# AppleHolic/pytorch_sound

Hardware: AMD Instinct MI355X
Metric: audio-sec/s STFT+mel+fwd/bwd (higher is better)
Workload: dtype bf16; 1 GPU; configs[1]: Conv1d separator (4 x ResBlock1, C=256, on 513-bin magnitude), 22.05 kHz, STFT 1024/256, 80 mel, batch 32 x 2 s per GPU, Adam, bf16 autocast; global_batch=32, parallelism=dp1, model_params=5520386

## Files before the change

include/psnd.h:

```cpp
#ifndef PSND_H
#define PSND_H

#include <stdint.h>
#include <stddef.h>

#ifdef __cplusplus
extern "C" {
#endif

#define PSND_OK 0
#define PSND_E_ARG (-1)
#define PSND_E_SHAPE (-2)
#define PSND_E_HIP (-3)
#define PSND_E_UNSUPPORTED (-4)

#define PSND_FRAMING_CENTER 0
#define PSND_FRAMING_HIFIGAN 1
#define PSND_FRAMING_NONE 2

int psnd_version(void);
const char *psnd_last_error(void);
#ifdef PSND_LAB
void psnd_env_refresh(void);
#endif
// ... 89 lines not shown
typedef struct psnd_chain_pair {
    const void *W1;
    const float *bias1;
    float act1_slope;
    void *mid_out;
    const void *W2;
    const float *bias2;
    int off1, dstep1, off2, dstep2;
    float act2_slope;
    void *out_raw, *out_act;
    const void *M1, *M2;
    float m1_slope, m2_slope;
} psnd_chain_pair;
int psnd_conv1d_cl_chain_rows(int C, int k, int n_pairs, const int *taps);
int psnd_conv1d_cl_chain_plan(int C, int k, int n_pairs, const int *taps, int64_t R, int *mr_out);
int psnd_conv1d_cl_chain(const void *A, const void *res, const psnd_chain_pair *pairs, int n_pairs, int64_t N, int Lp, int L, int HP,
                         int C, int k, void *stream);
void psnd_conv_chain_stats(long long *out2);
int psnd_to_cl_nfk(const float *x_nfk, int64_t N, int K, int64_t F, int Lp, int HP, int Cp, int preop, void *out, void *stream);
int64_t psnd_mask_head_l1_blocks_nfk(int64_t N, int64_t F, int K);
int psnd_mask_head_l1_fwd_nfk(const void *y, const float *mag_nfk, const float *ref_nfk, int64_t N, int K, int64_t F, int Lp, int HP, int Cp,
                              float *est_nfk, double *part, void *stream);
int psnd_mask_head_l1_bwd_nfk(const float *gest_nfk, const float *mag_nfk, const void *y, const float *est_nfk, const float *ref_nfk,
                              const float *g, float coef, int64_t N, int K, int64_t F, int Lp, int HP, int Cp, void *gy, void *stream);
int psnd_mel_fwd_nfk(const float *mag_nfk, int64_t N, int64_t F, int M, int K, const void *mel_plan, int log_kind, float log_offset,
                     float pre_clamp_min, float clamp_lo, float clamp_hi, float *out, float *mel_lin, void *stream);
int psnd_mel_bwd_nfk(const float *gout, const float *mel_lin, int64_t N, int64_t F, int M, int K, const void *mel_plan, int log_kind,
                     float log_offset, float pre_clamp_min, float clamp_lo, float clamp_hi, float *gmag_nfk, void *stream);
int psnd_mel_l1_fwd_nfk(const float *mag_nfk, int64_t N, int64_t F, int M, int K, const void *mel_plan, int log_kind, float log_offset,
                        float pre_clamp_min, float clamp_lo, float clamp_hi, const float *ref, float *mel_lin, double *part, void *stream);
int psnd_mel_l1_bwd_nfk(const float *ref, const float *mel_lin, const float *g, float coef, int64_t N, int64_t F, int M, int K,
                        const void *mel_plan, int log_kind, float log_offset, float pre_clamp_min, float clamp_lo, float clamp_hi,
                        float *gmag_nfk, void *stream);
int64_t psnd_mask_head_l1_blocks(int64_t N, int64_t T, int Cp);
int psnd_mask_head_l1_fwd(const void *y, const float *mag, const float *ref, int64_t N, int C, int64_t T, int Lp, int HP, int Cp,
                          float *est, double *part, void *stream);
int psnd_mask_head_l1_bwd(const float *gest, const float *mag, const void *y, const float *est, const float *ref, const float *g,
                          float coef, int64_t N, int C, int64_t T, int Lp, int HP, int Cp, void *gy, void *stream);
int64_t psnd_mel_l1_blocks(int64_t N, int64_t F, int M);
int psnd_mel_l1_fwd(const float *mag, int64_t N, int64_t F, int M, int K, const void *mel_plan, int log_kind, float log_offset,
                    float pre_clamp_min, float clamp_lo, float clamp_hi, const float *ref, float *mel_lin, double *part, void *stream);
int psnd_mel_l1_bwd(const float *ref, const float *mel_lin, const float *g, float coef, int64_t N, int64_t F, int M, int K,
                    const void *mel_plan, int log_kind, float log_offset, float pre_clamp_min, float clamp_lo, float clamp_hi,
                    float *gmag, void *stream);
int psnd_nan_flag(const float *x, int64_t n, float *flag, void *stream);
int psnd_l1_loss_combine(const double *const *parts, const int64_t *nb, const double *scale, int terms, float *out, float *nan_flag, void *stream);
int psnd_conv_stats(int64_t *out4, int reset);
int psnd_conv_pair_stats(int64_t *out4, int reset);
int psnd_conv1d_cl_wgrad(const void *G1, const void *G2, const void *GM, float g2_slope, const void *xa, int64_t N,
                         int Lp, int Ca, int Cb, int k, int off0, int dstep, float *gw_part, float *gbias_part,
                         void *g_out, void *stream);
int psnd_conv1d_prep(const float *v, const float *g, const float *bias, int Cout, int Cin, int k, int Cb, int Ca,
                     void *wf, void *wb, float *bias_padded, void *stream);
int psnd_convtr1d_prep(const float *v, const float *g, const float *bias, int Cin, int Cout, int K, int stride, int Cr, int Cip,
                       void *wf, void *wb, float *bias_rep, void *stream);
int psnd_convtr1d_prep_multi(const void *descs_dev, int n, int total_blocks, void *stream);
int psnd_convtr1d_cl_fwd(const void *xa, const void *wf, const float *bias_rep, int64_t N, int Lp, int L, int HP, int Cip, int Cr,
                         int stride, int padding, int LpO, int HPO, float act_slope, void *out_raw, void *out_act, void *stream);
int psnd_convtr1d_cl_wgrad_splits(int64_t N, int Lp, int Cip, int Cr, int stride);
int psnd_convtr1d_cl_bwd(const void *g_raw, const void *g_act, const void *act, float act_slope, const void *wb, const void *xa,
                         int64_t N, int Lp, int L, int HP, int Cip, int Cr, int stride, int padding, int LpO, int HPO, void *gx,
                         void *g_eff, float *gw_part, void *stream);
int psnd_convtr1d_wnorm_bwd(const float *gw_part, int splits, const float *v, const float *g, int Cin, int Cout, int K, int stride,
                            int Cr, int Cip, float *gv, float *gg, void *stream);
int psnd_cl_mean_act_fwd(const void *a, const void *b, const void *c, const void *d, int count, float slope, void *out, int64_t n,
                         void *stream);
// ... 175 lines not shown
```

pytorch_sound_amd/_lib.py:

```python
import ctypes
import os
import numpy as np

_HERE = os.path.dirname(os.path.abspath(__file__))
LIB_PATH = os.environ.get('PSND_LIB', os.path.join(_HERE, 'libpsnd_hip.so'))

PSND_OK = 0
FRAMING_CENTER = 0
FRAMING_HIFIGAN = 1
FRAMING_NONE = 2
LOG_NONE, LOG_E, LOG_10 = 0, 1, 2
MASK_NONE, MASK_LINEAR, MASK_SIGMOID = 0, 1, 2

_c = ctypes
_P = _c.c_void_p
_I64 = _c.c_int64
_INT = _c.c_int
_F = _c.c_float
_D = _c.c_double
_U32 = _c.c_uint32
_U64 = _c.c_uint64

SIGNATURES = {
    'psnd_version': (_INT, []),
# ... 30 lines not shown
    'psnd_conv1d_cl': (_INT, [_P, _P, _P, _F, _P, _P, _P, _P, _I64, _INT, _INT, _INT, _INT, _INT, _INT, _INT, _INT, _F, _F, _P, _P, _P, _P]),
    'psnd_conv1d_cl_pair_supported': (_INT, [_INT, _INT, _INT, _INT, _INT, _INT]),
    'psnd_conv1d_cl_pair': (_INT, [_P, _P, _P, _P, _F, _F, _P, _P, _P, _P, _F, _P, _I64, _INT, _INT, _INT, _INT, _INT, _INT, _INT, _INT, _INT, _F, _P, _P, _P]),
    'psnd_conv1d_cl_wgrad': (_INT, [_P, _P, _P, _F, _P, _I64, _INT, _INT, _INT, _INT, _INT, _INT, _P, _P, _P, _P]),
    'psnd_conv1d_prep': (_INT, [_P, _P, _P, _INT, _INT, _INT, _INT, _INT, _P, _P, _P, _P]),
    'psnd_conv1d_wnorm_bwd': (_INT, [_P, _P, _INT, _P, _P, _INT, _INT, _INT, _INT, _INT, _P, _P, _P, _P]),
    'psnd_conv1d_cl_bwd': (_INT, [_P, _P, _P, _F, _P, _P, _I64, _INT, _INT, _INT, _INT, _INT, _INT, _INT, _INT, _P, _P, _P, _F, _P, _P, _P, _P]),
    'psnd_conv1d_cl_wgrad_multi_splits': (_INT, [_I64, _INT, _INT, _INT, _INT, _INT]),
    'psnd_conv1d_cl_wgrad_multi': (_INT, [_P, _INT, _I64, _INT, _P]),
    'psnd_nan_flag': (_INT, [_P, _I64, _P, _P]),
    'psnd_conv1d_cl_chain_rows': (_INT, [_INT, _INT, _INT, _P]),
    'psnd_conv1d_cl_chain_plan': (_INT, [_INT, _INT, _INT, _P, _I64, _P]),
    'psnd_conv1d_cl_chain': (_INT, [_P, _P, _P, _INT, _I64, _INT, _INT, _INT, _INT, _INT, _P]),
    'psnd_conv_chain_stats': (None, [_P]),
    'psnd_conv1d_cl_pair_bwd_supported': (_INT, [_INT, _INT, _INT, _INT, _INT, _INT]),
    'psnd_conv1d_cl_pair_bwd_splits': (_INT, [_I64, _INT, _INT, _INT]),
    'psnd_conv1d_cl_pair_bwd': (_INT, [_P, _P, _P, _F, _P, _P, _P, _F, _P, _I64, _INT, _INT, _INT, _INT, _INT, _INT, _INT, _INT, _INT, _P, _P, _P, _P,
                                       _P, _P, _INT, _INT, _P, _P, _P]),
    'psnd_conv1d_wnorm_bwd_multi': (_INT, [_P, _INT, _P]),
    'psnd_conv1d_prep_multi': (_INT, [_P, _INT, _INT, _INT, _INT, _P]),
    'psnd_conv1d_cl_wgrad_splits': (_INT, [_I64, _INT, _INT, _INT, _INT]),
    'psnd_mask_head_l1_blocks': (_I64, [_I64, _I64, _INT]),
    'psnd_masked_l1_blocks': (_I64, [_I64]),
    'psnd_masked_l1_fwd': (_INT, [_P, _P, _P, _I64, _INT, _I64, _P, _P, _P, _P]),
    'psnd_masked_l1_bwd': (_INT, [_P, _P, _P, _I64, _INT, _I64, _P, _P, _P, _P, _P]),
    'psnd_to_cl_nfk': (_INT, [_P, _I64, _INT, _I64, _INT, _INT, _INT, _INT, _P, _P]),
    'psnd_mask_head_l1_blocks_nfk': (_I64, [_I64, _I64, _INT]),
    'psnd_mask_head_l1_fwd_nfk': (_INT, [_P, _P, _P, _I64, _INT, _I64, _INT, _INT, _INT, _P, _P, _P]),
    'psnd_mask_head_l1_bwd_nfk': (_INT, [_P, _P, _P, _P, _P, _P, _F, _I64, _INT, _I64, _INT, _INT, _INT, _P, _P]),
    'psnd_mel_fwd_nfk': (_INT, [_P, _I64, _I64, _INT, _INT, _P, _INT, _F, _F, _F, _F, _P, _P, _P]),
    'psnd_mel_bwd_nfk': (_INT, [_P, _P, _I64, _I64, _INT, _INT, _P, _INT, _F, _F, _F, _F, _P, _P]),
    'psnd_mel_l1_fwd_nfk': (_INT, [_P, _I64, _I64, _INT, _INT, _P, _INT, _F, _F, _F, _F, _P, _P, _P, _P]),
    'psnd_mel_l1_bwd_nfk': (_INT, [_P, _P, _P, _F, _I64, _I64, _INT, _INT, _P, _INT, _F, _F, _F, _F, _P, _P]),
    'psnd_mask_head_l1_fwd': (_INT, [_P, _P, _P, _I64, _INT, _I64, _INT, _INT, _INT, _P, _P, _P]),
    'psnd_mask_head_l1_bwd': (_INT, [_P, _P, _P, _P, _P, _P, _F, _I64, _INT, _I64, _INT, _INT, _INT, _P, _P]),
    'psnd_mel_l1_blocks': (_I64, [_I64, _I64, _INT]),
    'psnd_mel_l1_fwd': (_INT, [_P, _I64, _I64, _INT, _INT, _P, _INT, _F, _F, _F, _F, _P, _P, _P, _P]),
    'psnd_mel_l1_bwd': (_INT, [_P, _P, _P, _F, _I64, _I64, _INT, _INT, _P, _INT, _F, _F, _F, _F, _P, _P]),
    'psnd_l1_loss_combine': (_INT, [_P, _P, _P, _INT, _P, _P, _P]),
    'psnd_conv_stats': (_INT, [_P, _INT]),
    'psnd_conv_pair_stats': (_INT, [_P, _INT]),
    'psnd_convtr1d_prep_multi': (_INT, [_P, _INT, _INT, _P]),
    'psnd_convtr1d_prep': (_INT, [_P, _P, _P, _INT, _INT, _INT, _INT, _INT, _INT, _P, _P, _P, _P]),
    'psnd_convtr1d_cl_fwd': (_INT, [_P, _P, _P, _I64, _INT, _INT, _INT, _INT, _INT, _INT, _INT, _INT, _INT, _F, _P, _P, _P]),
    'psnd_convtr1d_cl_wgrad_splits': (_INT, [_I64, _INT, _INT, _INT, _INT]),
    'psnd_convtr1d_cl_bwd': (_INT, [_P, _P, _P, _F, _P, _P, _I64, _INT, _INT, _INT, _INT, _INT, _INT, _INT, _INT, _INT, _P, _P, _P, _P]),
    'psnd_convtr1d_wnorm_bwd': (_INT, [_P, _INT, _P, _P, _INT, _INT, _INT, _INT, _INT, _INT, _P, _P, _P]),
    'psnd_cl_mean_act_fwd': (_INT, [_P, _P, _P, _P, _INT, _F, _P, _I64, _P]),
    'psnd_cl_mean_act_bwd': (_INT, [_P, _P, _INT, _F, _P, _I64, _P]),
    'psnd_cl_sum2': (_INT, [_P, _INT, _P, _P, _INT, _P, _I64, _P]),
    'psnd_grad_pack_bf16': (_INT, [_P, _P, _I64, _F, _P]),
    'psnd_grad_unpack_bf16': (_INT, [_P, _P, _I64, _F, _P]),
    'psnd_cl_colsum_splits': (_INT, [_I64, _INT]),
    'psnd_cl_colsum': (_INT, [_P, _I64, _INT, _INT, _INT, _INT, _P, _P, _P]),
    'psnd_posenc': (_INT, [_P, _P, _F, _I64, _INT, _I64, _I64, _P, _P]),
    'psnd_groupnorm1_fwd': (_INT, [_P, _P, _P, _P, _I64, _INT, _I64, _F, _INT, _P, _P, _P, _P]),
    'psnd_groupnorm1_bwd': (_INT, [_P, _P, _P, _P, _P, _P, _I64, _INT, _I64, _INT, _P, _P, _P, _P, _P]),
    'psnd_groupnorm1_drop_fwd': (_INT, [_P, _P, _P, _P, _I64, _INT, _I64, _F, _INT, _P, _P, _P, _P, _U32, _F, _P]),
    'psnd_groupnorm1_drop_bwd': (_INT, [_P, _P, _P, _P, _P, _P, _I64, _INT, _I64, _INT, _P, _P, _P, _P, _P, _P, _U32, _F, _P]),
    'psnd_rng_seed': (_INT, [_P, _U64, _U64, _P]),
    'psnd_rng_next': (_INT, [_P, _P, _P]),
    'psnd_linear1x1_fwd': (_INT, [_P, _P, _P, _I64, _INT, _INT, _I64, _INT, _INT, _P, _P]),
    'psnd_linear1x1_wgrad_slabs': (_I64, [_I64, _INT, _INT, _I64]),
    'psnd_linear1x1_bwd': (_INT, [_P, _P, _P, _P, _I64, _INT, _INT, _I64, _INT, _P, _P, _P, _P, _P]),
    'psnd_linear1x1_bwd_acc': (_INT, [_P, _P, _P, _P, _I64, _INT, _INT, _I64, _INT, _P, _P, _P, _P, _P, _P]),
    'psnd_linear1x1_bwd_ex': (_INT, [_P, _P, _P, _P, _I64, _INT, _INT, _I64, _INT, _INT, _I64, _P, _P, _P, _P, _P, _P, _P]),
# ... 199 lines not shown
```

pytorch_sound_amd/cl.py:

```python
import ctypes
from collections import namedtuple
from pytorch_sound_amd import _switches as _sw
import weakref

import torch

from . import _lib
from ._lib import lib, check, ptr, stream_ptr

ALIGN_C = 32


def round_up(x, m):
    return (x + m - 1) // m * m


class CLShape:

    def __init__(self, N, L, HP):
        self.N, self.L, self.HP = int(N), int(L), int(HP)
        self.Lp = round_up(self.L + 2 * self.HP, 8)

    @property
    def R(self):
# ... 168 lines not shown
    def backward(ctx, g, _gest):
        y, mag, mag_ref, mel_ref, mel_plan, est, lin = ctx.saved_tensors
        shape, M, log_kind, log_offset, pre, lo, hi, c1, c2 = ctx.cfg
        N, C, T = mag.shape
        if g is None:
            return (None,) * 14
        g = g.contiguous().float()
        gest = torch.empty_like(mag)
        gy = torch.empty_like(y)
        st = stream_ptr(y.device)
        with torch.cuda.device(y.device):
            check(lib().psnd_mel_l1_bwd(ptr(mel_ref), ptr(lin), ptr(g), c2, N, T, M, C, ptr(mel_plan), log_kind, log_offset, pre, lo, hi,
                                        ptr(gest), st), 'psnd_mel_l1_bwd')
            check(lib().psnd_mask_head_l1_bwd(ptr(gest), ptr(mag), ptr(y), ptr(est), ptr(mag_ref), ptr(g), c1, N, C, T, shape.Lp, shape.HP,
                                              y.shape[2], ptr(gy), st), 'psnd_mask_head_l1_bwd')
        return (gy,) + (None,) * 13


def to_cl_nfk(x_nfk, shape, preop=0):
    _need(x_nfk, torch.float32)
    if x_nfk.requires_grad and torch.is_grad_enabled():
        raise _lib.PsndError('to_cl_nfk carries no gradient (feature tensors are inputs); use ToCL on an (N, K, F) tensor')
    N, F, K = x_nfk.shape
    if F != shape.L or N != shape.N:
        raise _lib.PsndError('to_cl_nfk: tensor %s does not match the CL geometry (N=%d, L=%d)' % (tuple(x_nfk.shape), shape.N, shape.L))
    Cp = round_up(K, ALIGN_C)
    out = torch.empty((N, shape.Lp, Cp), dtype=torch.bfloat16, device=x_nfk.device)
    with torch.cuda.device(x_nfk.device):
        check(lib().psnd_to_cl_nfk(ptr(x_nfk), N, K, F, shape.Lp, shape.HP, Cp, int(preop), ptr(out), stream_ptr(x_nfk.device)),
              'psnd_to_cl_nfk')
    return out


class MaskHeadSpectralL1NFK(torch.autograd.Function):

    @staticmethod
    def forward(ctx, y, mag, mag_ref, mel_ref, mel_plan, shape, M, log_kind, log_offset, pre_clamp_min, clamp_lo, clamp_hi, w1, w2):
        from .kernels import _clamp_args
        ctx.set_materialize_grads(False)
        _need(y, torch.bfloat16)
        for t in (mag, mag_ref, mel_ref):
            _need(t, torch.float32)
        N, F, K = mag.shape
        if mag_ref.shape != mag.shape or tuple(mel_ref.shape) != (N, M, F):
            raise _lib.PsndError('mask_head_spectral_l1 (nfk): mag_ref %s / mel_ref %s do not match mag %s and %d mel bands'
                                 % (tuple(mag_ref.shape), tuple(mel_ref.shape), tuple(mag.shape), M))
        dev = y.device
        lo, hi, pre = _clamp_args(clamp_lo, clamp_hi, pre_clamp_min)
        est = torch.empty_like(mag)
        lin = torch.empty((N, M, F), dtype=torch.float32, device=dev)
        nb1 = int(lib().psnd_mask_head_l1_blocks_nfk(N, F, K))
        nb2 = int(lib().psnd_mel_l1_blocks(N, F, M))
        part = torch.empty(nb1 + nb2, dtype=torch.float64, device=dev)
        out = torch.empty((), dtype=torch.float32, device=dev)
        st = stream_ptr(dev)
        with torch.cuda.device(dev):
            check(lib().psnd_mask_head_l1_fwd_nfk(ptr(y), ptr(mag), ptr(mag_ref), N, K, F, shape.Lp, shape.HP, y.shape[2], ptr(est),
                                                  ptr(part), st), 'psnd_mask_head_l1_fwd_nfk')
            p2 = ctypes.c_void_p(part.data_ptr() + 8 * nb1)
            check(lib().psnd_mel_l1_fwd_nfk(ptr(est), N, F, M, K, ptr(mel_plan), log_kind, float(log_offset), pre, lo, hi, ptr(mel_ref),
                                            ptr(lin), p2, st), 'psnd_mel_l1_fwd_nfk')
            parts = (ctypes.c_void_p * 2)(part.data_ptr(), part.data_ptr() + 8 * nb1)
            nbs = (ctypes.c_int64 * 2)(nb1, nb2)
            sc = (ctypes.c_double * 2)(float(w1) / mag.numel(), float(w2) / mel_ref.numel())
            nan_flag = _nan_flag_tensor(dev)
            check(lib().psnd_l1_loss_combine(parts, nbs, sc, 2, ptr(out), ptr(nan_flag), st), 'psnd_l1_loss_combine')
        LAST_LOSS_NAN_FLAG[0] = nan_flag
        ctx.cfg = (shape, M, log_kind, float(log_offset), pre, lo, hi, float(w1) / mag.numel(), float(w2) / mel_ref.numel())
        ctx.save_for_backward(y, mag, mag_ref, mel_ref, mel_plan, est, lin)
        ctx.mark_non_differentiable(est)
        return out, est

    @staticmethod
    def backward(ctx, g, _gest):
        y, mag, mag_ref, mel_ref, mel_plan, est, lin = ctx.saved_tensors
        shape, M, log_kind, log_offset, pre, lo, hi, c1, c2 = ctx.cfg
        N, F, K = mag.shape
        if g is None:
            return (None,) * 14
        g = g.contiguous().float()
        gest = torch.empty_like(mag)
        gy = torch.empty_like(y)
        st = stream_ptr(y.device)
        with torch.cuda.device(y.device):
            check(lib().psnd_mel_l1_bwd_nfk(ptr(mel_ref), ptr(lin), ptr(g), c2, N, F, M, K, ptr(mel_plan), log_kind, log_offset, pre, lo, hi,
                                            ptr(gest), st), 'psnd_mel_l1_bwd_nfk')
            check(lib().psnd_mask_head_l1_bwd_nfk(ptr(gest), ptr(mag), ptr(y), ptr(est), ptr(mag_ref), ptr(g), c1, N, K, F, shape.Lp,
                                                  shape.HP, y.shape[2], ptr(gy), st), 'psnd_mask_head_l1_bwd_nfk')
        return (gy,) + (None,) * 13


def _launch_conv(A, A2, AM, a2_slope, W, bias, res, mask_src, shape, Ca, Cb, k, off0, dstep, act_slope, mask_slope,
                 want_raw, want_act, a_eff_out=None):
    dev = W.device
    raw = torch.empty((shape.N, shape.Lp, Cb), dtype=torch.bfloat16, device=dev) if want_raw else None
    act = torch.empty((shape.N, shape.Lp, Cb), dtype=torch.bfloat16, device=dev) if want_act else None
    with torch.cuda.device(dev):
        check(lib().psnd_conv1d_cl(ptr(A), ptr(A2), ptr(AM), float(a2_slope), ptr(W), ptr(bias), ptr(res), ptr(mask_src),
                                   shape.N, shape.Lp, shape.L, shape.HP, Ca, Cb, k, off0, dstep, float(act_slope),
                                   float(mask_slope), ptr(raw), ptr(act), ptr(a_eff_out), stream_ptr(dev)), 'psnd_conv1d_cl')
    return raw, act


_JOIN_PENDING = {}


def _join_side_at_end_of_backward(dev, side):
    target = torch.cuda.current_stream(dev)
    pending = _JOIN_PENDING.setdefault(dev.index, [])
    if not any(t == target and sd == side for t, sd in pending):
        pending.append((target, side))

    def join():
# ... 968 lines not shown
```

pytorch_sound_amd/csrc/psnd_core.hip:

```cpp
#include "psnd_common.h"

static thread_local char g_err[512] = "";

void psnd_set_error(const char *fmt, ...) {
    va_list ap;
    va_start(ap, fmt);
    vsnprintf(g_err, sizeof(g_err), fmt, ap);
    va_end(ap);
}

extern "C" int psnd_version(void) { return 144; }

extern "C" const char *psnd_last_error(void) { return g_err; }

#ifdef PSND_LAB
std::atomic<int> g_psnd_env_gen{0};
extern "C" void psnd_env_refresh(void) { g_psnd_env_gen.fetch_add(1, std::memory_order_acq_rel); }
#endif

static inline int64_t pad_of(int n_fft, int hop, int framing) {
    if (framing == PSND_FRAMING_NONE) return 0;
    return framing == PSND_FRAMING_CENTER ? n_fft / 2 : (n_fft - hop) / 2;
}

extern "C" int64_t psnd_frame_count(int64_t T, int n_fft, int hop, int framing) {
    if (T <= 0 || n_fft <= 0 || hop <= 0) return 0;
    const int64_t L = T + 2 * pad_of(n_fft, hop, framing);
    if (L < n_fft) return 0;
    return (L - n_fft) / hop + 1;
}

extern "C" int64_t psnd_frame_sample_index(int64_t f, int m, int64_t T, int n_fft, int hop, int framing) {
    int64_t i = f * hop - pad_of(n_fft, hop, framing) + m;
    if (i < 0) i = -i;
    if (i >= T) i = 2 * (T - 1) - i;
    return i;
}

extern "C" void *psnd_event_create(void) {
    hipEvent_t ev = nullptr;
    if (hipEventCreateWithFlags(&ev, hipEventDisableTiming) != hipSuccess) {
        psnd_set_error("event_create: %s", hipGetErrorString(hipGetLastError()));
        return nullptr;
    }
// ... 96 lines not shown
```

pytorch_sound_amd/csrc/psnd_mel.hip:

```cpp
#include "psnd_common.h"
#include <math.h>
#include <string.h>
#include <vector>

namespace {

inline int hdr_ints(int MT, int KT) { return (8 + 2 * MT + 2 * KT + 63) & ~63; }

struct MelParams {
    const float *in0;
    const float *in1;
    const int *plan;
    float *out;
    float *lin;
    long long F;
    int N, R, Cc;
    int RT, CS;
    int band_off;
    int w_off;
    int nft;
    int log_kind;
    float log_offset, pre_clamp_min, clamp_lo, clamp_hi;
    const float *l1_ref;
    double *l1_part;
    const float *l1_g;
    float l1_coef;
    int wn_off, CS16;
    int seg_off;
};

__device__ __forceinline__ float log_grad(float mel, int kind, float off, float pre, float lo, float hi) {
    float pass = 1.f;
    float v = mel;
    if (pre >= 0.f) {
        if (v < pre) pass = 0.f;
        v = fmaxf(v, pre);
    }
    v += off;
    float y = v, d = 1.f;
    if (kind == PSND_LOG_E) {
        y = logf(v);
        d = 1.f / v;
    } else if (kind == PSND_LOG_10) {
        y = log10f(v);
        d = 0.43429448190325182765f / v;
    }
    if (y < lo || y > hi) pass = 0.f;
    return pass * d;
}

__device__ __forceinline__ float l1_log_grad(float mel, float ref, int kind, float off, float pre, float lo, float hi) {
    float pass = 1.f, v = mel;
    if (pre >= 0.f) {
        if (v < pre) pass = 0.f;
        v = fmaxf(v, pre);
    }
    v += off;
    float y = v, d = 1.f;
    if (kind == PSND_LOG_E) {
        y = logf(v);
        d = 1.f / v;
    } else if (kind == PSND_LOG_10) {
        y = log10f(v);
        d = 0.43429448190325182765f / v;
    }
    if (y < lo || y > hi) pass = 0.f;
    y = fminf(fmaxf(y, lo), hi);
    const float sg = y > ref ? 1.f : (y < ref ? -1.f : 0.f);
    return sg * pass * d;
}

__device__ __forceinline__ f32x4 load_b_raw(__amdgpu_buffer_rsrc_t r, int c, int Cc, long long f, long long F) {
    const unsigned off = (c < Cc && f < F) ? (unsigned)(((size_t)c * F + f) * sizeof(float)) : 0xffffffffu;
    return __builtin_bit_cast(f32x4, __builtin_amdgcn_raw_buffer_load_b128(r, (int)off, 0, 0));
}

template <bool BWD, bool NFK = false>
__global__ __launch_bounds__(256) void mel_kernel(MelParams p) {
    const int lane = threadIdx.x & 63;
    const long long wid = (long long)blockIdx.x * 4 + (threadIdx.x >> 6);
    const long long per_clip = (long long)p.nft * p.RT;
    if (wid >= per_clip * p.N) return;
    const int clip = (int)(wid / per_clip);
    const int rem = (int)(wid - (long long)clip * per_clip);
    const int ft = rem / p.RT, rt = rem - ft * p.RT;
    const long long F = p.F;
    const long long f = (long long)ft * 64 + 4 * (lane & 15);
    const int kk = lane >> 4;

    const int lo = p.plan[p.band_off + 2 * rt], hi = p.plan[p.band_off + 2 * rt + 1];
    const float *W = reinterpret_cast<const float *>(p.plan) + p.w_off + (size_t)rt * p.CS * 64 + lane;
    const int in_bytes = (int)((size_t)p.Cc * F * sizeof(float));
    const __amdgpu_buffer_rsrc_t r0 = make_uniform_rsrc(p.in0 + (size_t)clip * p.Cc * F, in_bytes);
    const __amdgpu_buffer_rsrc_t r1 = make_uniform_rsrc(BWD ? p.in1 + (size_t)clip * p.Cc * F : p.in0, BWD ? in_bytes : 0);
    const bool l1b = BWD && p.l1_g != nullptr;
    const float l1c = l1b ? p.l1_coef * p.l1_g[0] : 0.f;

    f32x4 acc0 = {0.f, 0.f, 0.f, 0.f}, acc1 = acc0, acc2 = acc0, acc3 = acc0;
    auto batch = [&](auto muc, int s0) __attribute__((always_inline)) {
        constexpr int MU = decltype(muc)::value;
        float a[MU];
        f32x4 b[MU], m[BWD ? MU : 1];
#pragma unroll
        for (int u = 0; u < MU; ++u) {
            const int c = s0 + u < hi ? 4 * (s0 + u) + kk : p.Cc;
            a[u] = W[(size_t)min(s0 + u, hi - 1) * 64];
            b[u] = load_b_raw(r0, c, p.Cc, f, F);
            if constexpr (BWD) m[u] = load_b_raw(r1, c, p.Cc, f, F);
        }
        if constexpr (BWD) {
// ... 7 lines not shown
                } else {
                    b[u].x *= log_grad(m[u].x, p.log_kind, p.log_offset, p.pre_clamp_min, p.clamp_lo, p.clamp_hi);
                    b[u].y *= log_grad(m[u].y, p.log_kind, p.log_offset, p.pre_clamp_min, p.clamp_lo, p.clamp_hi);
                    b[u].z *= log_grad(m[u].z, p.log_kind, p.log_offset, p.pre_clamp_min, p.clamp_lo, p.clamp_hi);
                    b[u].w *= log_grad(m[u].w, p.log_kind, p.log_offset, p.pre_clamp_min, p.clamp_lo, p.clamp_hi);
                }
                if (!(s0 + u < hi && 4 * (s0 + u) + kk < p.Cc)) b[u] = f32x4{0.f, 0.f, 0.f, 0.f};
            }
        }
#pragma unroll
        for (int u = 0; u < MU; ++u) {
            acc0 = __builtin_amdgcn_mfma_f32_16x16x4f32(a[u], b[u].x, acc0, 0, 0, 0);
            acc1 = __builtin_amdgcn_mfma_f32_16x16x4f32(a[u], b[u].y, acc1, 0, 0, 0);
            acc2 = __builtin_amdgcn_mfma_f32_16x16x4f32(a[u], b[u].z, acc2, 0, 0, 0);
            acc3 = __builtin_amdgcn_mfma_f32_16x16x4f32(a[u], b[u].w, acc3, 0, 0, 0);
        }
    };
#ifndef PSND_MEL_MU
#define PSND_MEL_MU 8
#endif
    constexpr int MU = BWD ? 4 : PSND_MEL_MU;
    int s0 = lo;
    for (; s0 + MU <= hi; s0 += MU) batch(std::integral_constant<int, MU>{}, s0);
    if constexpr (BWD) {
        const int rest = hi - s0;
        if (rest == 1) batch(std::integral_constant<int, 1>{}, s0);
        else if (rest == 2) batch(std::integral_constant<int, 2>{}, s0);
        else if (rest == 3) batch(std::integral_constant<int, 3>{}, s0);
    } else {
        if (s0 < hi) batch(std::integral_constant<int, MU>{}, s0);
    }
    const size_t obase = (size_t)clip * p.R * F;
    float l1acc = 0.f;
    if constexpr (BWD && NFK) {
        const int bin0 = 16 * rt + 4 * kk;
        const f32x4 accs[4] = {acc0, acc1, acc2, acc3};
#pragma unroll
        for (int j = 0; j < 4; ++j) {
            if (f + j >= F || bin0 >= p.R) continue;
            float *dst = p.out + obase + (size_t)(f + j) * p.R + bin0;
            if (bin0 + 3 < p.R) {
                *reinterpret_cast<f32x4_u *>(dst) = accs[j];
            } else {
                for (int r = 0; r < 4; ++r)
                    if (bin0 + r < p.R) dst[r] = accs[j][r];
            }
        }
        return;
    }
#pragma unroll
    for (int r = 0; r < 4; ++r) {
        const int row = 16 * rt + 4 * kk + r;
        if (row >= p.R) continue;
        f32x4 v = {acc0[r], acc1[r], acc2[r], acc3[r]};
        f32x4 y = v;
        if constexpr (!BWD) {
            y.x = fminf(fmaxf(log_apply(v.x, p.log_kind, p.log_offset, p.pre_clamp_min), p.clamp_lo), p.clamp_hi);
            y.y = fminf(fmaxf(log_apply(v.y, p.log_kind, p.log_offset, p.pre_clamp_min), p.clamp_lo), p.clamp_hi);
            y.z = fminf(fmaxf(log_apply(v.z, p.log_kind, p.log_offset, p.pre_clamp_min), p.clamp_lo), p.clamp_hi);
            y.w = fminf(fmaxf(log_apply(v.w, p.log_kind, p.log_offset, p.pre_clamp_min), p.clamp_lo), p.clamp_hi);
        }
        const size_t o = obase + (size_t)row * F + f;
        if constexpr (!BWD) {
            if (p.l1_ref) {
                if (f + 3 < F) {
                    const f32x4 rf = *reinterpret_cast<const f32x4_u *>(p.l1_ref + o);
                    l1acc += fabsf(y.x - rf.x) + fabsf(y.y - rf.y) + fabsf(y.z - rf.z) + fabsf(y.w - rf.w);
// ... 296 lines not shown
            if (any) {
                if (s < lo) lo = s;
                hi = s + 1;
            }
        }
        if (hi <= lo) lo = hi = 0;
        hdr[8 + 2 * h.MT + 2 * t] = lo, hdr[8 + 2 * h.MT + 2 * t + 1] = hi;
    }
    for (int t = 0; t < h.MT; ++t)
        for (int S = 0; S < h.KS16; ++S)
            for (int lane = 0; lane < 64; ++lane)
                for (int j = 0; j < 4; ++j)
                    fl[h.wn_off + (((size_t)t * h.KS16 + S) * 64 + lane) * 4 + j] = w(16 * t + (lane & 15), 16 * S + 4 * (lane >> 4) + j);
    {
        int *sg = hdr + h.seg_off;
        auto lo = [&](int t) { return hdr[8 + 2 * t]; };
        auto hi = [&](int t) { return hdr[8 + 2 * t + 1]; };
        bool banded = true;
        for (int t = 0; t + 1 < h.MT; ++t) banded &= lo(t) <= lo(t + 1) && hi(t) <= hi(t + 1) && hi(t) > lo(t) && hi(t + 1) > lo(t + 1);
        for (int t = 0; t + 2 < h.MT; ++t) banded &= hi(t) <= lo(t + 2);
        for (int t = 0; t < h.MT; ++t) {
            int s1b = lo(t), s1e = hi(t), s2b = 0, s2e = 0;
            if (banded) {
                if (t > 0 && hi(t - 1) > s1b) s1b = hi(t - 1);
                if (t + 1 < h.MT && lo(t + 1) < s1e) s2b = lo(t + 1), s2e = s1e, s1e = s2b;
                if (s1e < s1b) s1e = s1b;
            }
            sg[4 * t] = s1b, sg[4 * t + 1] = s1e, sg[4 * t + 2] = s2b, sg[4 * t + 3] = s2e;
        }
    }
    return PSND_OK;
}

static int mel_launch(bool bwd, const float *in0, const float *in1, int64_t N, int64_t F, int M, int K,
                      const void *plan, int log_kind, float log_offset, float pre, float lo, float hi,
                      float *out, float *lin, void *stream, const float *l1_ref = nullptr, double *l1_part = nullptr,
                      const float *l1_g = nullptr, float l1_coef = 0.f, bool nfk = false) {
    if (!in0 || !plan || (!out && !l1_ref) || (bwd && !in1)) PSND_FAIL(PSND_E_ARG, "mel: null pointer");
    if (M <= 0 || K <= 0 || N < 0 || F < 0) PSND_FAIL(PSND_E_SHAPE, "mel: M=%d K=%d N=%lld F=%lld", M, K, (long long)N, (long long)F);
    if (log_kind < PSND_LOG_NONE || log_kind > PSND_LOG_10) PSND_FAIL(PSND_E_ARG, "mel: log_kind=%d", log_kind);
    if (N == 0 || F == 0) return PSND_OK;
    if ((size_t)(M > K ? M : K) * (size_t)F * sizeof(float) >= ((size_t)1 << 31))
        PSND_FAIL(PSND_E_SHAPE, "mel: a clip of %lld frames exceeds the 2 GB buffer range of one clip's operand", (long long)F);
    const MelHostPlan h = mel_layout(M, K);
    MelParams p;
    p.in0 = in0, p.in1 = in1, p.plan = static_cast<const int *>(plan), p.out = out, p.lin = lin;
    p.F = F, p.N = (int)N;
    p.log_kind = log_kind, p.log_offset = log_offset, p.pre_clamp_min = pre, p.clamp_lo = lo, p.clamp_hi = hi;
    p.nft = (int)((F + 63) / 64);
    p.l1_ref = l1_ref, p.l1_part = l1_part, p.l1_g = l1_g, p.l1_coef = l1_coef;
    p.wn_off = h.wn_off, p.CS16 = h.KS16, p.seg_off = h.seg_off;
    if (!bwd) {
        p.R = M, p.Cc = K, p.RT = h.MT, p.CS = h.KS, p.band_off = 8, p.w_off = h.fw_off;
    } else {
        p.R = K, p.Cc = M, p.RT = h.KT, p.CS = h.MS, p.band_off = 8 + 2 * h.MT, p.w_off = h.bw_off;
    }
    const bool once = !bwd && !nfk && h.MT <= kOnceTiles;
    const long long waves = (long long)N * p.nft * p.RT;
    const long long blocks = (waves + 3) / 4;
    if (blocks >= (1ll << 31) || waves >= (1ll << 31)) PSND_FAIL(PSND_E_SHAPE, "mel: grid too large");
    hipStream_t s = static_cast<hipStream_t>(stream);
    if (nfk) {
        if (!bwd) hipLaunchKernelGGL(mel_fwd_nfk_kernel, dim3((unsigned)waves), dim3(256), 0, s, p);
        else hipLaunchKernelGGL((mel_kernel<true, true>), dim3((unsigned)blocks), dim3(256), 0, s, p);
    } else if (!bwd && once) {
        const long long ob = ((long long)N * p.nft + 3) / 4;
        if (h.MT <= 5) hipLaunchKernelGGL(mel_fwd_once_kernel<5>, dim3((unsigned)ob), dim3(256), 0, s, p);
        else hipLaunchKernelGGL(mel_fwd_once_kernel<8>, dim3((unsigned)ob), dim3(256), 0, s, p);
    } else if (!bwd) hipLaunchKernelGGL(mel_kernel<false>, dim3((unsigned)blocks), dim3(256), 0, s, p);
    else hipLaunchKernelGGL(mel_kernel<true>, dim3((unsigned)blocks), dim3(256), 0, s, p);
    PSND_CHECK_LAUNCH(bwd ? "mel_bwd" : "mel_fwd");
    return PSND_OK;
}

extern "C" int psnd_mel_fwd(const float *mag, int64_t N, int64_t F, int M, int K, const void *mel_plan,
                            int log_kind, float log_offset, float pre_clamp_min, float clamp_lo, float clamp_hi,
                            float *out, float *mel_lin, void *stream) {
    return mel_launch(false, mag, nullptr, N, F, M, K, mel_plan, log_kind, log_offset, pre_clamp_min, clamp_lo,
                      clamp_hi, out, mel_lin, stream);
}

extern "C" int psnd_mel_bwd(const float *gout, const float *mel_lin, int64_t N, int64_t F, int M, int K,
                            const void *mel_plan, int log_kind, float log_offset, float pre_clamp_min,
                            float clamp_lo, float clamp_hi, float *gmag, void *stream) {
    return mel_launch(true, gout, mel_lin, N, F, M, K, mel_plan, log_kind, log_offset, pre_clamp_min, clamp_lo,
                      clamp_hi, gmag, nullptr, stream);
}

extern "C" int64_t psnd_mel_l1_blocks(int64_t N, int64_t F, int M) {
    if (N <= 0 || F <= 0 || M <= 0) return 0;
    return N * ((F + 63) / 64) * ((M + 15) / 16);
}
extern "C" int psnd_mel_l1_fwd(const float *mag, int64_t N, int64_t F, int M, int K, const void *mel_plan, int log_kind, float log_offset,
                               float pre_clamp_min, float clamp_lo, float clamp_hi, const float *ref, float *mel_lin, double *part,
                               void *stream) {
    if (!ref || !mel_lin || !part) PSND_FAIL(PSND_E_ARG, "mel_l1_fwd: null ref / mel_lin / part");
// ... 2 lines not shown
}
extern "C" int psnd_mel_l1_bwd(const float *ref, const float *mel_lin, const float *g, float coef, int64_t N, int64_t F, int M, int K,
                               const void *mel_plan, int log_kind, float log_offset, float pre_clamp_min, float clamp_lo, float clamp_hi,
                               float *gmag, void *stream) {
    if (!g) PSND_FAIL(PSND_E_ARG, "mel_l1_bwd: null g");
    return mel_launch(true, ref, mel_lin, N, F, M, K, mel_plan, log_kind, log_offset, pre_clamp_min, clamp_lo, clamp_hi, gmag, nullptr,
                      stream, nullptr, nullptr, g, coef);
}

extern "C" int psnd_mel_fwd_nfk(const float *mag_nfk, int64_t N, int64_t F, int M, int K, const void *mel_plan, int log_kind, float log_offset,
                                float pre_clamp_min, float clamp_lo, float clamp_hi, float *out, float *mel_lin, void *stream) {
    return mel_launch(false, mag_nfk, nullptr, N, F, M, K, mel_plan, log_kind, log_offset, pre_clamp_min, clamp_lo, clamp_hi, out, mel_lin, stream,
                      nullptr, nullptr, nullptr, 0.f, true);
}
extern "C" int psnd_mel_bwd_nfk(const float *gout, const float *mel_lin, int64_t N, int64_t F, int M, int K, const void *mel_plan, int log_kind,
                                float log_offset, float pre_clamp_min, float clamp_lo, float clamp_hi, float *gmag_nfk, void *stream) {
    return mel_launch(true, gout, mel_lin, N, F, M, K, mel_plan, log_kind, log_offset, pre_clamp_min, clamp_lo, clamp_hi, gmag_nfk, nullptr, stream,
                      nullptr, nullptr, nullptr, 0.f, true);
}
extern "C" int psnd_mel_l1_fwd_nfk(const float *mag_nfk, int64_t N, int64_t F, int M, int K, const void *mel_plan, int log_kind, float log_offset,
                                   float pre_clamp_min, float clamp_lo, float clamp_hi, const float *ref, float *mel_lin, double *part,
                                   void *stream) {
    if (!ref || !mel_lin || !part) PSND_FAIL(PSND_E_ARG, "mel_l1_fwd_nfk: null ref / mel_lin / part");
    return mel_launch(false, mag_nfk, nullptr, N, F, M, K, mel_plan, log_kind, log_offset, pre_clamp_min, clamp_lo, clamp_hi, nullptr, mel_lin,
                      stream, ref, part, nullptr, 0.f, true);
}
extern "C" int psnd_mel_l1_bwd_nfk(const float *ref, const float *mel_lin, const float *g, float coef, int64_t N, int64_t F, int M, int K,
                                   const void *mel_plan, int log_kind, float log_offset, float pre_clamp_min, float clamp_lo, float clamp_hi,
                                   float *gmag_nfk, void *stream) {
    if (!g) PSND_FAIL(PSND_E_ARG, "mel_l1_bwd_nfk: null g");
    return mel_launch(true, ref, mel_lin, N, F, M, K, mel_plan, log_kind, log_offset, pre_clamp_min, clamp_lo, clamp_hi, gmag_nfk, nullptr,
                      stream, nullptr, nullptr, g, coef, true);
}
```

Before: 105,600 audio-s/s.

## Fuse mel L1 backward with mask-head L1 backward into one kernel epilogue

Result: no change. 108,100 audio-s/s (median of 3 runs) (+2.3%).

```diff
diff --git a/include/psnd.h b/include/psnd.h
--- a/include/psnd.h
+++ b/include/psnd.h
@@ -145,6 +145,10 @@
 int psnd_mel_l1_bwd_nfk(const float *ref, const float *mel_lin, const float *g, float coef, int64_t N, int64_t F, int M, int K,
                         const void *mel_plan, int log_kind, float log_offset, float pre_clamp_min, float clamp_lo, float clamp_hi,
                         float *gmag_nfk, void *stream);
+int psnd_mask_mel_l1_bwd_nfk(const float *mel_ref, const float *mel_lin, const float *mag_nfk, const void *y, const float *mag_ref_nfk,
+                             const float *g, float c1, float c2, int64_t N, int64_t F, int M, int K, const void *mel_plan, int log_kind,
+                             float log_offset, float pre_clamp_min, float clamp_lo, float clamp_hi, int Lp, int HP, int Cp, void *gy,
+                             void *stream);
 int64_t psnd_mask_head_l1_blocks(int64_t N, int64_t T, int Cp);
 int psnd_mask_head_l1_fwd(const void *y, const float *mag, const float *ref, int64_t N, int C, int64_t T, int Lp, int HP, int Cp,
                           float *est, double *part, void *stream);
diff --git a/pytorch_sound_amd/_lib.py b/pytorch_sound_amd/_lib.py
--- a/pytorch_sound_amd/_lib.py
+++ b/pytorch_sound_amd/_lib.py
@@ -86,6 +86,8 @@
     'psnd_mel_bwd_nfk': (_INT, [_P, _P, _I64, _I64, _INT, _INT, _P, _INT, _F, _F, _F, _F, _P, _P]),
     'psnd_mel_l1_fwd_nfk': (_INT, [_P, _I64, _I64, _INT, _INT, _P, _INT, _F, _F, _F, _F, _P, _P, _P, _P]),
     'psnd_mel_l1_bwd_nfk': (_INT, [_P, _P, _P, _F, _I64, _I64, _INT, _INT, _P, _INT, _F, _F, _F, _F, _P, _P]),
+    'psnd_mask_mel_l1_bwd_nfk': (_INT, [_P, _P, _P, _P, _P, _P, _F, _F, _I64, _I64, _INT, _INT, _P, _INT, _F, _F, _F, _F, _INT, _INT, _INT,
+                                        _P, _P]),
     'psnd_mask_head_l1_fwd': (_INT, [_P, _P, _P, _I64, _INT, _I64, _INT, _INT, _INT, _P, _P, _P]),
     'psnd_mask_head_l1_bwd': (_INT, [_P, _P, _P, _P, _P, _P, _F, _I64, _INT, _I64, _INT, _INT, _INT, _P, _P]),
     'psnd_mel_l1_blocks': (_I64, [_I64, _I64, _INT]),
diff --git a/pytorch_sound_amd/cl.py b/pytorch_sound_amd/cl.py
--- a/pytorch_sound_amd/cl.py
+++ b/pytorch_sound_amd/cl.py
@@ -224,6 +224,9 @@
     return out
 
 
+FUSED_LOSS_TAIL = True
+
+
 class MaskHeadSpectralL1NFK(torch.autograd.Function):
 
     @staticmethod
@@ -259,18 +262,31 @@
             check(lib().psnd_l1_loss_combine(parts, nbs, sc, 2, ptr(out), ptr(nan_flag), st), 'psnd_l1_loss_combine')
         LAST_LOSS_NAN_FLAG[0] = nan_flag
         ctx.cfg = (shape, M, log_kind, float(log_offset), pre, lo, hi, float(w1) / mag.numel(), float(w2) / mel_ref.numel())
-        ctx.save_for_backward(y, mag, mag_ref, mel_ref, mel_plan, est, lin)
+        ctx.fused = bool(FUSED_LOSS_TAIL)
+        if ctx.fused:
+            ctx.save_for_backward(y, mag, mag_ref, mel_ref, mel_plan, lin)
+        else:
+            ctx.save_for_backward(y, mag, mag_ref, mel_ref, mel_plan, est, lin)
         ctx.mark_non_differentiable(est)
         return out, est
 
     @staticmethod
     def backward(ctx, g, _gest):
-        y, mag, mag_ref, mel_ref, mel_plan, est, lin = ctx.saved_tensors
-        shape, M, log_kind, log_offset, pre, lo, hi, c1, c2 = ctx.cfg
-        N, F, K = mag.shape
         if g is None:
             return (None,) * 14
+        shape, M, log_kind, log_offset, pre, lo, hi, c1, c2 = ctx.cfg
         g = g.contiguous().float()
+        if ctx.fused:
+            y, mag, mag_ref, mel_ref, mel_plan, lin = ctx.saved_tensors
+            N, F, K = mag.shape
+            gy = torch.empty_like(y)
+            with torch.cuda.device(y.device):
+                check(lib().psnd_mask_mel_l1_bwd_nfk(ptr(mel_ref), ptr(lin), ptr(mag), ptr(y), ptr(mag_ref), ptr(g), c1, c2, N, F, M, K,
+                                                     ptr(mel_plan), log_kind, log_offset, pre, lo, hi, shape.Lp, shape.HP, y.shape[2],
+                                                     ptr(gy), stream_ptr(y.device)), 'psnd_mask_mel_l1_bwd_nfk')
+            return (gy,) + (None,) * 13
+        y, mag, mag_ref, mel_ref, mel_plan, est, lin = ctx.saved_tensors
+        N, F, K = mag.shape
         gest = torch.empty_like(mag)
         gy = torch.empty_like(y)
         st = stream_ptr(y.device)
diff --git a/pytorch_sound_amd/csrc/psnd_core.hip b/pytorch_sound_amd/csrc/psnd_core.hip
--- a/pytorch_sound_amd/csrc/psnd_core.hip
+++ b/pytorch_sound_amd/csrc/psnd_core.hip
@@ -9,7 +9,7 @@
     va_end(ap);
 }
 
-extern "C" int psnd_version(void) { return 144; }
+extern "C" int psnd_version(void) { return 145; }
 
 extern "C" const char *psnd_last_error(void) { return g_err; }
 
diff --git a/pytorch_sound_amd/csrc/psnd_mel.hip b/pytorch_sound_amd/csrc/psnd_mel.hip
--- a/pytorch_sound_amd/csrc/psnd_mel.hip
+++ b/pytorch_sound_amd/csrc/psnd_mel.hip
@@ -27,7 +27,20 @@
     float l1_coef;
     int wn_off, CS16;
     int seg_off;
+    const float *mh_mag, *mh_ref;
+    const unsigned short *mh_y;
+    unsigned short *mh_gy;
+    float mh_coef;
+    int Lp, HP, Cp;
 };
+
+typedef __bf16 mel_hwbf16x2 __attribute__((ext_vector_type(2)));
+__device__ __forceinline__ float mel_bf_lo(unsigned v) { return __builtin_bit_cast(float, v << 16); }
+__device__ __forceinline__ float mel_bf_hi(unsigned v) { return __builtin_bit_cast(float, v & 0xffff0000u); }
+__device__ __forceinline__ unsigned mel_pack_bf16(float lo, float hi) {
+    const f32x2 v = {lo, hi};
+    return __builtin_bit_cast(unsigned, __builtin_convertvector(v, mel_hwbf16x2));
+}
 
 __device__ __forceinline__ float log_grad(float mel, int kind, float off, float pre, float lo, float hi) {
     float pass = 1.f;
@@ -75,7 +88,7 @@
     return __builtin_bit_cast(f32x4, __builtin_amdgcn_raw_buffer_load_b128(r, (int)off, 0, 0));
 }
 
-template <bool BWD, bool NFK = false>
+template <bool BWD, bool NFK = false, bool MASK = false>
 __global__ __launch_bounds__(256) void mel_kernel(MelParams p) {
     const int lane = threadIdx.x & 63;
     const long long wid = (long long)blockIdx.x * 4 + (threadIdx.x >> 6);
@@ -149,7 +162,77 @@
     }
     const size_t obase = (size_t)clip * p.R * F;
     float l1acc = 0.f;
-    if constexpr (BWD && NFK) {
+    if constexpr (BWD && NFK && MASK) {
+        constexpr unsigned OOB = 0xffffffffu;
+        const int K = p.R, Cp = p.Cp;
+        const int bin0 = 16 * rt + 4 * kk;
+        const int nfk_bytes = (int)((size_t)K * F * sizeof(float));
+        const int cl_bytes = (int)((size_t)p.Lp * Cp * 2);
+        const __amdgpu_buffer_rsrc_t rm = make_uniform_rsrc(p.mh_mag + (size_t)clip * K * F, nfk_bytes);
+        const __amdgpu_buffer_rsrc_t rr = make_uniform_rsrc(p.mh_ref + (size_t)clip * K * F, nfk_bytes);
+        const __amdgpu_buffer_rsrc_t ry = make_uniform_rsrc(p.mh_y + (size_t)clip * p.Lp * Cp, cl_bytes);
+        const __amdgpu_buffer_rsrc_t rg = make_uniform_rsrc(p.mh_gy + (size_t)clip * p.Lp * Cp, cl_bytes);
+        const float c1 = p.mh_coef * p.l1_g[0];
+        const bool whole = 16 * rt + 16 <= K;
+        const f32x4 accs[4] = {acc0, acc1, acc2, acc3};
+        f32x4 mg[4], rf[4];
+        u32x2 yq[4];
+        unsigned cb[4];
+#pragma unroll
+        for (int j = 0; j < 4; ++j) {
+            const bool ok = f + j < F;
+            const unsigned eb = ok ? (unsigned)((((size_t)(f + j)) * K + bin0) * sizeof(float)) : OOB;
+            cb[j] = (ok && bin0 + 4 <= Cp) ? (unsigned)((((size_t)(p.HP + f + j)) * Cp + bin0) * 2) : OOB;
+            if (whole) {
+                mg[j] = __builtin_bit_cast(f32x4, __builtin_amdgcn_raw_buffer_load_b128(rm, (int)eb, 0, 0));
+                rf[j] = __builtin_bit_cast(f32x4, __builtin_amdgcn_raw_buffer_load_b128(rr, (int)eb, 0, 0));
+            } else {
+#pragma unroll
+                for (int e = 0; e < 4; ++e) {
+                    const unsigned o = (ok && bin0 + e < K) ? eb + 4u * e : OOB;
+                    mg[j][e] = __builtin_bit_cast(float, __builtin_amdgcn_raw_buffer_load_b32(rm, (int)o, 0, 0));
+                    rf[j][e] = __builtin_bit_cast(float, __builtin_amdgcn_raw_buffer_load_b32(rr, (int)o, 0, 0));
+                }
+            }
+            yq[j] = __builtin_bit_cast(u32x2, __builtin_amdgcn_raw_buffer_load_b64(ry, (int)cb[j], 0, 0));
+        }
+#pragma unroll
+        for (int j = 0; j < 4; ++j) {
+            float w[4];
+#pragma unroll
+            for (int e = 0; e < 4; ++e) {
+                const unsigned q = yq[j][e >> 1];
+                const float yv = (e & 1) ? mel_bf_hi(q) : mel_bf_lo(q);
+                const float est = mg[j][e] / (1.f + __expf(-yv));
+                const float sg = 1.f / (1.f + __expf(-yv));
+                const float d = est - rf[j][e];
+                const float gg = accs[j][e] + c1 * (d > 0.f ? 1.f : (d < 0.f ? -1.f : 0.f));
+                w[e] = gg * mg[j][e] * sg * (1.f - sg);
+            }
+            const u32x2 o = {mel_pack_bf16(w[0], w[1]), mel_pack_bf16(w[2], w[3])};
+            __builtin_amdgcn_raw_buffer_store_b64(o, rg, (int)cb[j], 0, 0);
+        }
+        const u32x2 z2 = {0u, 0u};
+        const bool last = rt == p.RT - 1;
+        if (last) {
+            const int c0 = 16 * p.RT, np = (Cp - c0) >> 2;
+            for (int i = lane; i < 64 * np; i += 64) {
+                const long long fr = (long long)ft * 64 + i / np;
+                const int pc = i % np;
+                if (fr < F) __builtin_amdgcn_raw_buffer_store_b64(z2, rg, (int)(unsigned)((((size_t)(p.HP + fr)) * Cp + c0 + 4 * pc) * 2), 0, 0);
+            }
+        }
+        if (ft == 0) {
+            const int c0 = 16 * rt, c1e = last ? Cp : min(c0 + 16, Cp), np = (c1e - c0) >> 2;
+            const int nh = p.Lp - (int)F;
+            for (int i = lane; i < nh * np; i += 64) {
+                const int h = i / np, pc = i % np;
+                const long long l = h < p.HP ? h : h + F;
+                __builtin_amdgcn_raw_buffer_store_b64(z2, rg, (int)(unsigned)((((size_t)l) * Cp + c0 + 4 * pc) * 2), 0, 0);
+            }
+        }
+        return;
+    } else if constexpr (BWD && NFK) {
         const int bin0 = 16 * rt + 4 * kk;
         const f32x4 accs[4] = {acc0, acc1, acc2, acc3};
 #pragma unroll
@@ -512,11 +595,19 @@
     return PSND_OK;
 }
 
+struct MaskEpilogue {
+    const float *mag, *ref;
+    const void *y;
+    void *gy;
+    float coef;
+    int Lp, HP, Cp;
+};
+
 static int mel_launch(bool bwd, const float *in0, const float *in1, int64_t N, int64_t F, int M, int K,
                       const void *plan, int log_kind, float log_offset, float pre, float lo, float hi,
                       float *out, float *lin, void *stream, const float *l1_ref = nullptr, double *l1_part = nullptr,
-                      const float *l1_g = nullptr, float l1_coef = 0.f, bool nfk = false) {
-    if (!in0 || !plan || (!out && !l1_ref) || (bwd && !in1)) PSND_FAIL(PSND_E_ARG, "mel: null pointer");
+                      const float *l1_g = nullptr, float l1_coef = 0.f, bool nfk = false, const MaskEpilogue *mh = nullptr) {
+    if (!in0 || !plan || (!out && !l1_ref && !mh) || (bwd && !in1)) PSND_FAIL(PSND_E_ARG, "mel: null pointer");
     if (M <= 0 || K <= 0 || N < 0 || F < 0) PSND_FAIL(PSND_E_SHAPE, "mel: M=%d K=%d N=%lld F=%lld", M, K, (long long)N, (long long)F);
     if (log_kind < PSND_LOG_NONE || log_kind > PSND_LOG_10) PSND_FAIL(PSND_E_ARG, "mel: log_kind=%d", log_kind);
     if (N == 0 || F == 0) return PSND_OK;
@@ -530,6 +621,11 @@
     p.nft = (int)((F + 63) / 64);
     p.l1_ref = l1_ref, p.l1_part = l1_part, p.l1_g = l1_g, p.l1_coef = l1_coef;
     p.wn_off = h.wn_off, p.CS16 = h.KS16, p.seg_off = h.seg_off;
+    p.mh_mag = p.mh_ref = nullptr, p.mh_y = nullptr, p.mh_gy = nullptr, p.mh_coef = 0.f, p.Lp = p.HP = p.Cp = 0;
+    if (mh) {
+        p.mh_mag = mh->mag, p.mh_ref = mh->ref, p.mh_y = static_cast<const unsigned short *>(mh->y), p.mh_gy = static_cast<unsigned short *>(mh->gy);
+        p.mh_coef = mh->coef, p.Lp = mh->Lp, p.HP = mh->HP, p.Cp = mh->Cp;
+    }
     if (!bwd) {
         p.R = M, p.Cc = K, p.RT = h.MT, p.CS = h.KS, p.band_off = 8, p.w_off = h.fw_off;
     } else {
@@ -542,6 +638,7 @@
     hipStream_t s = static_cast<hipStream_t>(stream);
     if (nfk) {
         if (!bwd) hipLaunchKernelGGL(mel_fwd_nfk_kernel, dim3((unsigned)waves), dim3(256), 0, s, p);
+        else if (mh) hipLaunchKernelGGL((mel_kernel<true, true, true>), dim3((unsigned)blocks), dim3(256), 0, s, p);
         else hipLaunchKernelGGL((mel_kernel<true, true>), dim3((unsigned)blocks), dim3(256), 0, s, p);
     } else if (!bwd && once) {
         const long long ob = ((long long)N * p.nft + 3) / 4;
@@ -610,3 +707,17 @@
     return mel_launch(true, ref, mel_lin, N, F, M, K, mel_plan, log_kind, log_offset, pre_clamp_min, clamp_lo, clamp_hi, gmag_nfk, nullptr,
                       stream, nullptr, nullptr, g, coef, true);
 }
+
+extern "C" int psnd_mask_mel_l1_bwd_nfk(const float *mel_ref, const float *mel_lin, const float *mag_nfk, const void *y, const float *mag_ref_nfk,
+                                        const float *g, float c1, float c2, int64_t N, int64_t F, int M, int K, const void *mel_plan, int log_kind,
+                                        float log_offset, float pre_clamp_min, float clamp_lo, float clamp_hi, int Lp, int HP, int Cp, void *gy,
+                                        void *stream) {
+    if (!mel_ref || !mel_lin || !mag_nfk || !y || !mag_ref_nfk || !g || !mel_plan || !gy) PSND_FAIL(PSND_E_ARG, "mask_mel_l1_bwd_nfk: null pointer");
+    if (N < 0 || K <= 0 || M <= 0 || F <= 0 || HP < 0 || Lp < F + 2 * (int64_t)HP || Cp < ((K + 7) & ~7) || Cp % 8 != 0 ||
+        (size_t)N * (size_t)K * (size_t)F * 4 >= ((size_t)1 << 32) - 64 || (size_t)Lp * Cp * 2 >= ((size_t)1 << 31) ||
+        N * (int64_t)Lp * (Cp / 8) >= ((int64_t)1 << 39))
+        PSND_FAIL(PSND_E_SHAPE, "mask_mel_l1_bwd_nfk: N=%lld F=%lld M=%d K=%d Lp=%d HP=%d Cp=%d", (long long)N, (long long)F, M, K, Lp, HP, Cp);
+    const MaskEpilogue mh = {mag_nfk, mag_ref_nfk, y, gy, c1, Lp, HP, Cp};
+    return mel_launch(true, mel_ref, mel_lin, N, F, M, K, mel_plan, log_kind, log_offset, pre_clamp_min, clamp_lo, clamp_hi, nullptr, nullptr,
+                      stream, nullptr, nullptr, g, c2, true, &mh);
+}
```
